# maxwellsh/DIGDriver

Measured on NVIDIA B200. Metric: genome_bases_scanned_per_s, higher is better.
Workload: dtype u8 bases -> int32 counts; f64 p-values

## Files before the change

digdriver_b200/csrc/scan_lb.cu:

```cuda
#include <cuda.h>
#include <string.h>

#include "scan_common.cuh"

using namespace digscan;

namespace {

constexpr int LB_CW = 16;
constexpr int LB_WW = 4;
constexpr int LB_PW = 4;
constexpr int LB_THREADS = (LB_CW + LB_WW + LB_PW) * 32;
constexpr int LB_CONS = LB_CW * 32;
constexpr int LB_SPAN = 128;
constexpr int LB_CHUNK = LB_CW * LB_SPAN;
constexpr uint32_t LB_DSTRIDE = (LB_CHUNK + 64) / 4;
constexpr uint32_t LB_MSTRIDE = (LB_CHUNK + 128) / 8;
constexpr uint32_t LB_DROW = LB_DSTRIDE + 16u;
constexpr uint32_t LB_MROW = LB_MSTRIDE + 16u;
constexpr uint32_t LB_DGROUP = 4u * LB_DROW;
constexpr uint32_t LB_MGROUP = 4u * LB_MROW;
static_assert(LB_DGROUP % 128u == 0u && LB_MGROUP % 128u == 0u, "groups start 128-byte aligned (TMA box destination)");
constexpr uint32_t LB_MBASE = 8u * LB_DGROUP;
constexpr uint32_t LB_STAGE_BYTES = 8u * (LB_DGROUP + LB_MGROUP);
// ... 13 lines not shown
constexpr int LB_NOUT = LB_WW;
constexpr uint32_t OFF_TRI = OFF_OUT + LB_NOUT * OUT_BYTES;
constexpr uint32_t TRI_BYTES = 64u * 33u * 4u;
constexpr uint32_t OFF_EXC = OFF_TRI + TRI_BYTES;
constexpr uint32_t EXC_BYTES = 2048u;
constexpr uint32_t OFF_CNT = OFF_EXC + 2u * EXC_BYTES;
constexpr uint32_t OFF_CHK = OFF_CNT + 256u;
constexpr uint32_t OFF_FLG = OFF_CHK + 128u;
constexpr uint32_t OFF_BAR = OFF_FLG + 16u;
constexpr uint32_t LB_SMEM = OFF_BAR + 256u;
static_assert(OFF_BAR % 16u == 0u, "barrier block alignment");
static_assert(LB_SMEM <= 232448u, "shared memory budget");

constexpr uint32_t LB_BSTAGE = 8u * LB_DGROUP;
constexpr uint32_t OFF_SUM = OFF_STG + 3u * LB_BSTAGE;
static_assert(OFF_SUM + 4u * 128u <= OFF_OUT && LB_BSTAGE <= LB_NOUT * OUT_BYTES, "bases-only ring layout");

enum { BAR_FULL = 0, BAR_EMPTY = 2, BAR_OUTFULL = 4, BAR_OUTEMPTY = 8, BAR_DONE = 12, BAR_CLEAN = 13 };

#ifndef DIG_LB_STAGE3
#define DIG_LB_STAGE3 1
#endif
constexpr bool LB_ST3 = DIG_LB_STAGE3 != 0;
enum { BAR_FULL2 = 14, BAR_EMPTY2 = 15, BAR_OUTFREE = 16, BAR_FULL3 = 17, BAR_EMPTY3 = 18 };
__device__ __forceinline__ uint32_t lb3_full(uint32_t stage)
{
    return stage < 2u ? (uint32_t)BAR_FULL + stage : (stage == 2u ? (uint32_t)BAR_FULL2 : (uint32_t)BAR_FULL3);
}
__device__ __forceinline__ uint32_t lb3_empty(uint32_t stage)
{
    return stage < 2u ? (uint32_t)BAR_EMPTY + stage : (stage == 2u ? (uint32_t)BAR_EMPTY2 : (uint32_t)BAR_EMPTY3);
}
template <bool NS>
struct LbSlots {
    static constexpr uint32_t N = NS ? 4u : 3u;
};
template <bool NS>
__device__ __forceinline__ uint32_t lb_slot(uint32_t stg0, uint32_t stage)
{
    if constexpr (NS) return stage < 3u ? stg0 + stage * LB_BSTAGE : stg0 + (OFF_OUT - OFF_STG);
    else return stg0 + stage * LB_STAGE_BYTES;
}
__device__ __forceinline__ uint32_t lb_slot_sum(uint32_t stg0, uint32_t stage) { return stg0 + (OFF_SUM - OFF_STG) + stage * 128u; }

template <int GM>
struct LbRing {
    static constexpr uint32_t NST = 2u, LOG = 1u, STG0 = OFF_STG, FULL0 = BAR_FULL, EMPTY0 = BAR_EMPTY;
};
constexpr uint32_t TRI_TAB_BYTES = 256u * 128u;
template <>
struct LbRing<2> {
    static constexpr uint32_t NST = 4u, LOG = 2u, STG0 = TRI_TAB_BYTES, FULL0 = 0u, EMPTY0 = 4u;
};
template <>
struct LbRing<3> {
    static constexpr uint32_t NST = 2u, LOG = 1u, STG0 = 0u , FULL0 = 0u, EMPTY0 = 2u;
};
// ... 348 lines not shown

__device__ __forceinline__ int lb_chunk_order(int kq, int nch) { return kq == 0 ? nch - 1 : kq - 1; }

struct LbMaps {
    CUtensorMap d[2], m[2];
};

template <int GM, bool NS>
__device__ __forceinline__ void lb_producer(const LbArgs &A, const LbMaps *maps, const LbTeam T, int pw, int lane)
{
    const uint32_t bar = T.bar;
    const int64_t n_batches = (A.n_reg + 31) >> 5;
    const int m = lane & 3;
    const bool mine = (lane >> T.lane_shift) == pw;
    uint32_t ci = 0u;
    constexpr bool ST3 = LB_ST3 && GM < 2;
    constexpr uint32_t NSL = LbSlots<NS>::N;
    uint32_t uses = 0u, pbi = 0u;
    for (int64_t b = T.b0; b < n_batches; b += T.bstep, ++pbi) {
        const LbGeom g = lb_geom<GM>(b * 32 + lb_win(lane), A.n_reg, A.chrom_off, A.chrom_len, A.reg_chrom, A.reg_start, A.reg_end);
        const int nch = warp_max(g.nch);
        uint32_t st3 = 0u;
        if constexpr (ST3) {
            if (pbi >= 2u) mbar_wait_idle(bar + 8u * BAR_OUTFREE, pbi & 1u);
        }
        const int lead = lane & ~3;
        const uint32_t olo = __shfl_sync(0xffffffffu, (uint32_t)(unsigned long long)g.O, lead);
        const uint32_t ohi = __shfl_sync(0xffffffffu, (uint32_t)((unsigned long long)g.O >> 32), lead);
        const int64_t O0 = (int64_t)(((unsigned long long)ohi << 32) | olo);
        const int n0 = __shfl_sync(0xffffffffu, g.nch, lead);
        const bool fits = A.tile_w > 0 && g.nch > 0 && g.nch == n0 && O0 >= 0 && g.O == O0 + (int64_t)m * 8 * A.tile_w &&
                          g.O + (int64_t)g.nch * LB_CHUNK + 128 <= A.n_bases;
        const uint32_t okm = __ballot_sync(0xffffffffu, fits);
        const bool regular = ((okm >> lead) & 0xFu) == 0xFu;
        const uint32_t ped = (uint32_t)(A.tile_w >> 1), pem = (uint32_t)(A.tile_w >> 2);
        uint32_t xd0 = 0u, yd0 = 0u, xm0 = 0u, ym0 = 0u;
        if (regular && m == 0) {
            const uint32_t ed = (uint32_t)(O0 >> 4), em = (uint32_t)(O0 >> 5);
            yd0 = ed / ped; xd0 = ed - yd0 * ped;
            ym0 = em / pem; xm0 = em - ym0 * pem;
// ... 9 lines not shown
                uses ^= 1u << stage;
                full_i = lb3_full(stage);
                empty_i = lb3_empty(stage);
            } else {
                stage = ci & (R::NST - 1u);
                fpar = (ci >> R::LOG) & 1u;
                full_i = R::FULL0 + stage;
                empty_i = R::EMPTY0 + stage;
            }
            uint32_t sw = 0u;
            if constexpr (NS) {
                if (mine && k < g.nch) sw = lb_span_states(A.nsum, A.n_bases, g.O + (int64_t)k * LB_CHUNK);
            }
            LB_T(t_e0);
            mbar_wait_idle(bar + 8u * empty_i, fpar ^ 1u);
            if constexpr (ST3) {
                if (stage == NSL - 1u && pbi >= 1u) mbar_wait_idle(bar + 8u * BAR_OUTFREE, (pbi - 1u) & 1u);
            }
            LB_T(t_e1);
            const uint32_t full = bar + 8u * full_i;
            const uint32_t stg = ST3 ? lb_slot<NS>(T.stg0, stage) : T.stg0 + stage * LB_STAGE_BYTES;
            if constexpr (NS) {
                if (mine) sts32((ST3 ? lb_slot_sum(T.stg0, stage) : stg + LB_MBASE) + (uint32_t)lb_win(lane) * 4u, sw);
            }
            if (!mine) {
            } else if (regular && k < g.nch) {
                if (m == 0) {
                    uint32_t xd = xd0 + 128u * (uint32_t)k, yd = yd0, xm = xm0 + 64u * (uint32_t)k, ym = ym0;
                    if (xd >= ped) { xd -= ped; ++yd; }
                    if (xm >= pem) { xm -= pem; ++ym; }
                    const int lead = ((lane >> 2) & 1) * 4;
                    int bxd = (int)xd - lead, bxm = (int)xm - lead, sd = 0, sm = 0;
                    if (bxd + (int)(LB_DROW / 4) > (int)ped) { bxd -= (int)A.dshift; sd = 1; }
// ... 33 lines not shown
                    atomicAdd(A.timing + 12, (unsigned long long)(t_i - t_e1));
                }
            }
#endif
        }
    }
}

template <bool TRI, bool NS>
__device__ __forceinline__ void lb_consumer(const LbArgs &A, uint32_t sbase, int warp, int lane)
{
    constexpr uint32_t NSL = LbSlots<NS>::N;
    const uint32_t bar = sbase + OFF_BAR;
    const uint32_t tabl = sbase + OFF_TAB + (uint32_t)lane * 4u;
    const int64_t n_batches = (A.n_reg + 31) >> 5;
    uint32_t cit = 0u, bi = 0u, uses = 0u;
    const uint32_t top_r = A.top | (tabl & A.zero);
    const int grp = warp >> 3, w8 = warp & 7;
#ifdef DIG_LB_TIMING
    unsigned long long tacc[16] = {0, 0, 0, 0, 0, 0, 0, 0, 0, 0, 0, 0, 0, 0, 0, 0};
#endif
    LB_T(t_k0);
    LbGeom gnext = lb_geom<TRI>((int64_t)blockIdx.x * 32 + lb_win(lane), A.n_reg, A.chrom_off, A.chrom_len, A.reg_chrom, A.reg_start, A.reg_end);
    for (int64_t b = blockIdx.x; b < n_batches; b += gridDim.x, ++bi) {
        LB_T(t_g0);
        const LbGeom g = gnext;
        const int nch = warp_max(g.nch);
        LB_T(t_g1);
        LB_ACC(13, t_g0, t_g1);
        const uint32_t par = bi & 1u;
        const uint32_t exc = sbase + OFF_EXC + par * EXC_BYTES;
        uint32_t npairs = 0u;
        bool clean = bi == 0u;
        uint32_t st3 = 0u;
        for (int kq = 0; kq < nch; ++kq, ++cit) {
            const int k = lb_chunk_order(kq, nch);
            uint32_t stage, fpar, full_i, empty_i;
            if constexpr (LB_ST3) {
                stage = st3;
                st3 = st3 == NSL - 1u ? 0u : st3 + 1u;
                fpar = (uses >> stage) & 1u;
                uses ^= 1u << stage;
                full_i = lb3_full(stage);
                empty_i = lb3_empty(stage);
            } else {
                stage = cit & 1u;
                fpar = (cit >> 1) & 1u;
                full_i = BAR_FULL + stage;
                empty_i = BAR_EMPTY + stage;
            }
            LB_T(t_a);
            mbar_wait(bar + 8u * full_i, fpar);
            LB_T(t_b);
            LB_ACC(0, t_a, t_b);
            LB_ACC((kq == 0 ? 8 : (kq == 1 ? 9 : 10)), t_a, t_b);
            const uint32_t stg = LB_ST3 ? lb_slot<NS>(sbase + OFF_STG, stage) : sbase + OFF_STG + stage * LB_STAGE_BYTES;
            {
                const int base0 = k * LB_CHUNK + warp * LB_SPAN;
                const int lo_u = TRI ? min(g.lo5, g.lo3) : g.lo5, hi_u = TRI ? max(g.hi5, g.hi3) : g.hi5;
                if (!__any_sync(0xffffffffu, k < g.nch && lo_u - base0 < 130 && hi_u - base0 > 2)) {
                    if (lane == 0) mbar_arrive(bar + 8u * empty_i);
                    continue;
                }
            }
            const uint32_t dptr = stg + lb_dstrip(lane) + (uint32_t)warp * 32u;
            uint32_t D[9], M[5] = {0u, 0u, 0u, 0u, 0u}, sst = 0u;
            uint32_t dep;
            {
                const uint4 a = lds128(dptr), c = lds128(dptr + 16u);
                D[0] = a.x; D[1] = a.y; D[2] = a.z; D[3] = a.w;
                D[4] = c.x; D[5] = c.y; D[6] = c.z; D[7] = c.w;
                D[8] = lds32(dptr + 32u);
                if constexpr (NS) {
                    const uint32_t sa = LB_ST3 ? lb_slot_sum(sbase + OFF_STG, stage) : stg + LB_MBASE;
                    sst = (lds32(sa + (uint32_t)lb_win(lane) * 4u) >> (2 * warp)) & 3u;
                    dep = (D[0] | D[4]) ^ (D[8] | sst);
                } else {
                    const uint32_t mptr = stg + lb_mstrip(lane) + (uint32_t)warp * 16u;
                    const uint4 m = lds128(mptr);
                    M[0] = m.x; M[1] = m.y; M[2] = m.z; M[3] = m.w;
                    M[4] = lds32(mptr + 16u);
                    dep = (D[0] | D[4]) ^ (D[8] | M[0]) ^ M[4];
                }
            }
            __syncwarp();
            if (lane == 0) mbar_arrive_after_loads(bar + 8u * empty_i, dep, A.zero);
            if (!clean) {
                LB_T(t_c);
                mbar_wait(bar + 8u * BAR_CLEAN, (bi - 1u) & 1u);
                LB_T(t_d);
                LB_ACC(1, t_c, t_d);
                clean = true;
            }
            LB_T(t_p0);
            const int base = k * LB_CHUNK + warp * LB_SPAN;
            const int lo5 = g.lo5 - base, hi5 = g.hi5 - base;
            const uint32_t any_n = NS ? sst : M[0] | M[1] | M[2] | M[3] | (M[4] & 0xF0000000u);
            uint32_t PV[4] = {0u, 0u, 0u, 0u};
#ifdef DIG_LB_UNIFORM_PATH
            if (__all_sync(0xffffffffu, any_n == 0u && lo5 <= 2 && hi5 >= 130)) {
#else
            if (any_n == 0u && lo5 <= 2 && hi5 >= 130) {
#endif
                lb_pairs<false>(D, tabl, A.k32, top_r, PV);
                npairs += 64u;
            } else if (k < g.nch && (!NS || sst != 3u)) {
                if constexpr (NS) {
                    if (sst != 0u) lb_mask_global(A.nmask, A.n_bases, g.O + base, M);
// ... 20 lines not shown
                        if (pos < (uint32_t)LB_EXC_CAP) sts32(exc + 16u + 4u * pos, ((uint32_t)lane << 16) | key);
                    }
                    while (x3) {
                        const int t = __clz(x3);
                        x3 &= ~(0x80000000u >> t);
                        const uint32_t key = lb_bits(D, 32 * j + t + 1, 6);
                        const uint32_t pos = atom_add(exc, 1u);
                        if (pos < (uint32_t)LB_EXC_CAP) sts32(exc + 16u + 4u * pos, ((uint32_t)lane << 16) | 0x8000u | key);
                    }
                }
                if ((PV[0] | PV[1] | PV[2] | PV[3]) != 0u) lb_pairs<true>(D, tabl, A.k32, top_r, PV);
            }
            LB_T(t_p1);
            LB_ACC(2, t_p0, t_p1);
        }
        if (!clean) mbar_wait(bar + 8u * BAR_CLEAN, (bi - 1u) & 1u);
        if (npairs) red_add(sbase + OFF_CNT + par * 128u + (uint32_t)lane * 4u, npairs);
        LB_T(t_s0);
        cons_sync();
        LB_T(t_s1);
        LB_ACC(3, t_s0, t_s1);
        const int64_t rn = (b + gridDim.x) * 32 + lb_win(lane);
        const bool nact = b + gridDim.x < n_batches && rn < A.n_reg;
        int32_t nc = 0;
        int64_t nrs = 0, nre = 0;
        if (nact) {
            nc = __ldg(A.reg_chrom + rn);
            nrs = __ldg(A.reg_start + rn);
            nre = __ldg(A.reg_end + rn);
        }
        mbar_wait(bar + 8u * BAR_DONE, (bi & 1u) ^ 1u);
        LB_T(t_s2);
        LB_ACC(4, t_s1, t_s2);

        uint32_t tri_acc[4] = {0u, 0u, 0u, 0u};
#pragma unroll 1
        for (int i2 = 0; i2 < 4; ++i2) {
          if (i2 == 1) gnext = lb_geom2<TRI>(nact, nc, nrs, nre, A.chrom_off, A.chrom_len);
#pragma unroll
          for (int h = 0; h < 2; ++h) {
            const int i = 2 * i2 + h;
            const int sg = 2 * i + grp;
            const uint32_t buf = (uint32_t)(sg & 3);
            const uint32_t outb = sbase + OFF_OUT + buf * OUT_BYTES + (uint32_t)lb_win(lane) * 256u;
            LB_T(t_w0);
            mbar_wait(bar + 8u * (BAR_OUTEMPTY + buf), (((bi << 2) + (uint32_t)(sg >> 2)) & 1u) ^ 1u);
            LB_T(t_w1);
            LB_ACC(5, t_w0, t_w1);
#pragma unroll
            for (int t = 0; t < 2; ++t) {
                const int jl = (2 * w8 + t + lane) & 15;
                const int j = 16 * sg + jl;
                const uint32_t k0 = lds32(tabl + (uint32_t)(4 * j + 0) * 128u), k1 = lds32(tabl + (uint32_t)(4 * j + 1) * 128u);
                const uint32_t k2 = lds32(tabl + (uint32_t)(4 * j + 2) * 128u), k3 = lds32(tabl + (uint32_t)(4 * j + 3) * 128u);
                const uint32_t w0 = lds32(tabl + (uint32_t)(j)*128u), w1 = lds32(tabl + (uint32_t)(256 + j) * 128u);
                const uint32_t w2 = lds32(tabl + (uint32_t)(512 + j) * 128u), w3 = lds32(tabl + (uint32_t)(768 + j) * 128u);
                const uint32_t a0 = __dp4a(k0, 0x01010101u, 0u), a1 = __dp4a(k1, 0x01010101u, 0u);
                const uint32_t a2 = __dp4a(k2, 0x01010101u, 0u), a3 = __dp4a(k3, 0x01010101u, 0u);
                const uint32_t o0 = __dp4a(w3, 0x01000000u, __dp4a(w2, 0x01000000u, __dp4a(w1, 0x01000000u, __dp4a(w0, 0x01000000u, a0))));
                const uint32_t o2 = __dp4a(w3, 0x00000100u, __dp4a(w2, 0x00000100u, __dp4a(w1, 0x00000100u, __dp4a(w0, 0x00000100u, a2))));
                const uint32_t ev = ((w0 & 0x00FF00FFu) + (w1 & 0x00FF00FFu)) + ((w2 & 0x00FF00FFu) + (w3 & 0x00FF00FFu));
                const uint32_t o1 = a1 + (ev >> 16), o3 = a3 + (ev & 0xFFFFu);
                sts128(outb + (uint32_t)jl * 16u, o0, o1, o2, o3);
                tri_acc[2 * h + t] += (o0 + o1) + (o2 + o3);
            }
            if (i2 == 3) {
                if constexpr (TRI) {
#pragma unroll
                    for (int t = 0; t < 2; ++t) {
                        const uint32_t bin = (uint32_t)(16 * (sg & 3) + ((2 * w8 + t + lane) & 15));
                        red_add(sbase + OFF_TRI + (bin * 33u + (uint32_t)lane) * 4u, tri_acc[2 * h + t]);
                    }
                }
                if (h == 1) red_add(sbase + OFF_CHK + (uint32_t)lane * 4u, (tri_acc[0] + tri_acc[1]) + (tri_acc[2] + tri_acc[3]));
            }
            fence_async();
            __syncwarp();
            if (lane == 0) mbar_arrive(bar + 8u * (BAR_OUTFULL + buf));
            LB_T(t_w2);
            LB_ACC(6, t_w1, t_w2);
          }
        }
    }
#ifdef DIG_LB_TIMING
    LB_T(t_k1);
    LB_ACC(14, t_k0, t_k1);
    if (A.timing != nullptr && lane == 0) {
#pragma unroll
        for (int q = 0; q < 15; ++q)
            if (q != 7 && q != 11 && q != 12) atomicAdd(A.timing + q, tacc[q]);
    }
#endif
}

template <bool TRI, bool TOT>
__device__ __forceinline__ void lb_writer(const LbArgs &A, const CUtensorMap *tmap, uint32_t sbase, int q, int lane)
{
    const uint32_t bar = sbase + OFF_BAR;
    const int64_t n_batches = (A.n_reg + 31) >> 5;
    uint32_t use = 0u, bi = 0u;
    unsigned int tot5[TOT ? 8 : 1], tot3[2] = {0u, 0u};
#pragma unroll
    for (int i = 0; i < (TOT ? 8 : 1); ++i) tot5[i] = 0u;
    unsigned int acc_kb = 0u;
    const uint32_t out = sbase + OFF_OUT + (uint32_t)q * OUT_BYTES;

    auto flush_totals = [&]() {
        if constexpr (TOT) {
#pragma unroll
            for (int i = 0; i < 8; ++i) {
                if (tot5[i]) atomicAdd(A.totals5 + 64 * (4 * (i >> 1) + q) + 2 * lane + (i & 1), (unsigned long long)tot5[i]);
                tot5[i] = 0u;
            }
            if constexpr (TRI) {
                if (tot3[0]) atomicAdd(A.totals3 + lane, (unsigned long long)tot3[0]);
                if (tot3[1]) atomicAdd(A.totals3 + 32 + lane, (unsigned long long)tot3[1]);
                tot3[0] = tot3[1] = 0u;
            }
        }
    };

    for (int64_t b = blockIdx.x; b < n_batches; b += gridDim.x, ++bi) {
        const LbGeom g = lb_geom<TRI>(b * 32 + lb_win(lane), A.n_reg, A.chrom_off, A.chrom_len, A.reg_chrom, A.reg_start, A.reg_end);
        const uint32_t par = bi & 1u;
        const uint32_t exc = sbase + OFF_EXC + par * EXC_BYTES;
        const int64_t r = b * 32 + lb_win(lane);
        unsigned int tmp5[TOT ? 8 : 1], tmp3[2] = {0u, 0u};
#pragma unroll
        for (int i = 0; i < (TOT ? 8 : 1); ++i) tmp5[i] = 0u;
        uint32_t n_exc_raw = 0u;
#pragma unroll
        for (int s4 = 0; s4 < 4; ++s4, ++use) {
            const int sg = 4 * s4 + q;
            mbar_wait_idle(bar + 8u * (BAR_OUTFULL + q), use & 1u);
            if (s4 == 0) n_exc_raw = lds32(exc);
            const uint32_t n_exc = n_exc_raw < (uint32_t)LB_EXC_CAP ? n_exc_raw : (uint32_t)LB_EXC_CAP;
            for (uint32_t e = lane; e < n_exc; e += 32u) {
                const uint32_t ent = lds32(exc + 16u + 4u * e);
                if (!(ent & 0x8000u) && ((ent & 1023u) >> 6) == (uint32_t)sg)
                    red_add(out + (uint32_t)lb_win((int)(ent >> 16)) * 256u + (ent & 63u) * 4u, 1u);
            }
            fence_async();
            __syncwarp();
            if (lane == 0) {
                tensor_s2g(tmap, out, 64 * sg, (int)(b * 32));
                bulk_commit();
            }
            if constexpr (TOT) {
#pragma unroll 8
                for (int l2 = 0; l2 < 32; ++l2) {
                    const uint2 v = lds64(out + (uint32_t)l2 * 256u + (uint32_t)lane * 8u);
                    tmp5[2 * s4] += v.x;
                    tmp5[2 * s4 + 1] += v.y;
                }
            }
            uint32_t dep = 0u;
            if constexpr (TOT) dep = tmp5[2 * s4] | tmp5[2 * s4 + 1];
            __syncwarp();
            if (lane == 0) {
                bulk_wait_read<0>();
                mbar_arrive_after_loads(bar + 8u * (BAR_OUTEMPTY + q), dep, A.zero);
                if constexpr (LB_ST3) {
                    if (s4 == 3) mbar_arrive_after_loads(bar + 8u * BAR_OUTFREE, dep, A.zero);
                }
            }
            __syncwarp();
        }
        writer_sync();
#pragma unroll 8
        for (int i = 0; i < 64; ++i)
            sts128(sbase + OFF_TAB + (uint32_t)q * 32768u + (uint32_t)(lane + 32 * i) * 16u, 0u, 0u, 0u, 0u);
        __threadfence_block();
        __syncwarp();
        if (lane == 0) mbar_arrive(bar + 8u * BAR_CLEAN);
        if (q == 0) {
            const uint32_t n_exc = n_exc_raw < (uint32_t)LB_EXC_CAP ? n_exc_raw : (uint32_t)LB_EXC_CAP;
            if constexpr (TRI) {
                const uint32_t tri = sbase + OFF_TRI;
                for (uint32_t e = lane; e < n_exc; e += 32u) {
                    const uint32_t ent = lds32(exc + 16u + 4u * e);
                    const uint32_t bin = (ent & 0x8000u) ? (ent & 63u) : ((ent >> 2) & 63u);
                    red_add(tri + (bin * 33u + (ent >> 16)) * 4u, 1u);
                }
                __syncwarp();
#pragma unroll 4
                for (int l2 = 0; l2 < 32; ++l2) {
                    const int64_t r2 = b * 32 + lb_win(l2);
                    const uint32_t v0 = lds32(tri + ((uint32_t)lane * 33u + (uint32_t)l2) * 4u);
                    const uint32_t v1 = lds32(tri + ((uint32_t)(lane + 32) * 33u + (uint32_t)l2) * 4u);
                    if (r2 < A.n_reg) {
                        lb_store_tri(A, r2 * 64 + lane, (int)v0);
                        lb_store_tri(A, r2 * 64 + 32 + lane, (int)v1);
                    }
                    tmp3[0] += v0;
                    tmp3[1] += v1;
                }
                __syncwarp();
#pragma unroll 6
                for (int i = 0; i < 66; ++i) sts32(tri + (uint32_t)(lane + 32 * i) * 4u, 0u);
            }
            const uint32_t cnt_a = sbase + OFF_CNT + par * 128u + (uint32_t)lane * 4u, chk_a = sbase + OFF_CHK + (uint32_t)lane * 4u;
            const bool bad = 2u * lds32(cnt_a) != lds32(chk_a);
            const bool fail = __any_sync(0xffffffffu, bad) || n_exc_raw > (uint32_t)LB_EXC_CAP;
            sts32(cnt_a, 0u);
            sts32(chk_a, 0u);
            if (lane == 0) {
                sts32(exc, 0u);
                sts32(sbase + OFF_FLG, fail ? 1u : 0u);
            }
            if (g.too_long || (fail && g.active)) {
                const int pos = atomicAdd(A.fb_count, 1);
                A.fb_list[pos] = (int32_t)r;
            }
        }
        writer_sync();
        const bool fail = lds32(sbase + OFF_FLG) != 0u;
        if constexpr (TOT) {
            if (!fail) {
                unsigned int kb = g.nch > 0 ? (unsigned int)(g.nch * (LB_CHUNK >> 10)) : 0u;
#pragma unroll
                for (int o = 16; o > 0; o >>= 1) kb += __shfl_xor_sync(0xffffffffu, kb, o);
                if (acc_kb + kb > A.tot_limit_kb || acc_kb + kb < acc_kb) {
                    flush_totals();
                    acc_kb = 0u;
                }
                acc_kb += kb;
#pragma unroll
                for (int i = 0; i < 8; ++i) tot5[i] += tmp5[i];
                tot3[0] += tmp3[0];
                tot3[1] += tmp3[1];
            }
        }
        writer_sync();
        if (q == 0 && lane == 0) mbar_arrive(bar + 8u * BAR_DONE);
    }
    flush_totals();
    bulk_wait_all();
}

template <bool PRED>
__device__ __forceinline__ void lb_pairs4(const uint32_t (&D)[9], uint32_t tabl, uint32_t k128, const uint32_t (&PV)[4])
{
#pragma unroll
    for (int i = 0; i < 64; ++i) {
        const int q = i >> 3, off = 4 * (i & 7);
        uint32_t r;
        if (off <= 20) r = D[q] >> (22 - off);
        else r = __funnelshift_r(D[q + 1], D[q], 54 - off);
        uint32_t addr;
        asm("mad.lo.u32 %0, %1, %2, %3;" : "=r"(addr) : "r"(r & 0xFFu), "r"(k128), "r"(tabl));
        if constexpr (!PRED) {
            red_add(addr, 1u);
// ... 275 lines not shown
        const int ww = warp - LB_CW;
        lb_writer_tri<TOT, TEAMS>(A, sbase, ww / L::WW, ww % L::WW, lane);
    } else {
        lb_consumer_tri<TEAMS, NS>(A, sbase, warp / L::CW, warp % L::CW, lane);
    }
}

template <bool TRI, bool TOT, bool NS>
__global__ void __launch_bounds__(LB_THREADS, 1) scan_lb_kernel(const LbArgs A, const __grid_constant__ CUtensorMap tmap,
                                                                const __grid_constant__ LbMaps imaps)
{
    extern __shared__ __align__(1024) unsigned char smem_raw[];
    const uint32_t sbase = (uint32_t)__cvta_generic_to_shared(smem_raw);
    const int lane = threadIdx.x & 31;
    const int warp = __shfl_sync(0xffffffffu, threadIdx.x >> 5, 0);
    if ((sbase & 127u) != 0u) __trap();

    for (uint32_t i = threadIdx.x; i < OFF_BAR / 16u; i += LB_THREADS) sts128(sbase + i * 16u, 0u, 0u, 0u, 0u);
    if (threadIdx.x == 0) {
        const uint32_t bar = sbase + OFF_BAR;
        mbar_init(bar + 8u * (BAR_FULL + 0), 32u);
        mbar_init(bar + 8u * (BAR_FULL + 1), 32u);
        mbar_init(bar + 8u * (BAR_EMPTY + 0), LB_CW);
        mbar_init(bar + 8u * (BAR_EMPTY + 1), LB_CW);
        mbar_init(bar + 8u * BAR_FULL2, 32u);
        mbar_init(bar + 8u * BAR_EMPTY2, LB_CW);
        mbar_init(bar + 8u * BAR_FULL3, 32u);
        mbar_init(bar + 8u * BAR_EMPTY3, LB_CW);
        mbar_init(bar + 8u * BAR_OUTFREE, LB_WW);
#pragma unroll
        for (int i = 0; i < LB_NOUT; ++i) {
            mbar_init(bar + 8u * (BAR_OUTFULL + i), LB_CW / 2);
            mbar_init(bar + 8u * (BAR_OUTEMPTY + i), 1u);
        }
        mbar_init(bar + 8u * BAR_DONE, 1u);
        mbar_init(bar + 8u * BAR_CLEAN, LB_WW);
        asm volatile("fence.mbarrier_init.release.cluster;" ::: "memory");
        fence_async();
    }
    __syncthreads();
    if (warp >= LB_CW + LB_WW)
        lb_producer<TRI, NS>(A, &imaps, LbTeam{(int64_t)blockIdx.x, (int64_t)gridDim.x, sbase + OFF_BAR, sbase + LbRing<TRI>::STG0, 3},
                         warp - LB_CW - LB_WW, lane);
    else if (warp >= LB_CW) lb_writer<TRI, TOT>(A, &tmap, sbase, warp - LB_CW, lane);
    else lb_consumer<TRI, NS>(A, sbase, warp, lane);
}

typedef CUresult (*LbEncodeFn)(CUtensorMap *, CUtensorMapDataType, cuuint32_t, void *, const cuuint64_t *, const cuuint64_t *,
                               const cuuint32_t *, const cuuint32_t *, CUtensorMapInterleave, CUtensorMapSwizzle,
                               CUtensorMapL2promotion, CUtensorMapFloatOOBfill);

int lb_encode(CUtensorMap *tmap, CUtensorMapDataType dtype, const void *base, uint64_t dim0, uint64_t dim1, uint64_t pitch,
              uint32_t box0, uint32_t box1)
{
    static LbEncodeFn encode = nullptr;
    if (encode == nullptr) {
        void *fn = nullptr;
        cudaDriverEntryPointQueryResult q;
        DIG_CUDA(cudaGetDriverEntryPoint("cuTensorMapEncodeTiled", &fn, cudaEnableDefault, &q));
        if (fn == nullptr || q != cudaDriverEntryPointSuccess) {
            dig::set_error("%s: cuTensorMapEncodeTiled is not available", __func__);
            return DIG_ERR_CUDA;
        }
        encode = reinterpret_cast<LbEncodeFn>(fn);
    }
    const cuuint64_t gdim[2] = {dim0, dim1};
    const cuuint64_t gstride[1] = {pitch};
    const cuuint32_t box[2] = {box0, box1};
    const cuuint32_t estride[2] = {1u, 1u};
    const CUresult rc = encode(tmap, dtype, 2u, const_cast<void *>(base), gdim, gstride, box, estride, CU_TENSOR_MAP_INTERLEAVE_NONE,
                               CU_TENSOR_MAP_SWIZZLE_NONE, CU_TENSOR_MAP_L2_PROMOTION_NONE, CU_TENSOR_MAP_FLOAT_OOB_FILL_NONE);
    if (rc != CUDA_SUCCESS) {
        dig::set_error("%s: cuTensorMapEncodeTiled failed (%d)", __func__, (int)rc);
        return DIG_ERR_CUDA;
    }
    return DIG_OK;
}

int lb_tensor_map(CUtensorMap *tmap, int32_t *counts5, int64_t n_reg)
{
    return lb_encode(tmap, CU_TENSOR_MAP_DATA_TYPE_INT32, counts5, 1024u, (uint64_t)n_reg, 4096u, 64u, 32u);
}

int lb_input_maps(LbMaps *maps, LbArgs &A, int64_t tile_w)
{
    A.tile_w = 0;
    A.dshift = A.mshift = 0;
    memset(maps, 0, sizeof(*maps));
    if (tile_w < 4096 || (tile_w & 15) != 0 || tile_w > (int64_t)LB_MAX_CHUNKS * LB_CHUNK || A.n_bases >= ((int64_t)1 << 35))
        return DIG_OK;
    const uint64_t dbytes = (uint64_t)A.n_bases >> 2, mbytes = (uint64_t)A.n_bases >> 3;
    const uint64_t dpitch = 2u * (uint64_t)tile_w, mpitch = (uint64_t)tile_w;
    const uint64_t dsh = (dpitch / 2) & ~(uint64_t)15, msh = (mpitch / 2) & ~(uint64_t)15;
    if (dbytes <= dsh + dpitch || mbytes <= msh + mpitch) return DIG_OK;
    const unsigned char *p2b = reinterpret_cast<const unsigned char *>(A.p2);
    const unsigned char *nmb = reinterpret_cast<const unsigned char *>(A.nmask);
// ... 145 lines not shown
```

Measured before the change: 2828 billion.

## Snapshot count table into tensor memory and let writers reduce from TMEM

Consumers no longer reduce the shared count table into output tiles themselves. After each batch one thread snapshots the table into Blackwell tensor memory with tcgen05.cp, the consumers zero the table, and the writer warps read the counts from TMEM, reduce them and store them through 64B-swizzled TMA tiles. This takes the reduction off the consumer critical path and drops the OUTFULL/OUTEMPTY/CLEAN/OUTFREE handshakes, freeing one ring stage. It also rebalances registers with setmaxnreg and reorganises the exception and totals handling. It relies on one CTA per SM, a 512-column TMEM allocation and new descriptor layouts, and an error there would go unnoticed until the outputs are checked.

Result: slower. 2765 billion (median of 6 runs) (-2.2%).

```diff
diff --git a/digdriver_b200/csrc/lb_tmem.cuh b/digdriver_b200/csrc/lb_tmem.cuh
--- /dev/null
+++ b/digdriver_b200/csrc/lb_tmem.cuh
@@ -0,0 +1,62 @@
+#pragma once
+#include <stdint.h>
+
+namespace lbtmem {
+
+constexpr uint32_t COLS = 512;
+constexpr uint32_t START_COL = 256;
+
+__device__ __forceinline__ void alloc(uint32_t dst_smem)
+{
+    asm volatile("tcgen05.alloc.cta_group::1.sync.aligned.shared::cta.b32 [%0], %1;" ::"r"(dst_smem), "n"(COLS) : "memory");
+    asm volatile("tcgen05.relinquish_alloc_permit.cta_group::1.sync.aligned;" ::: "memory");
+}
+__device__ __forceinline__ void dealloc(uint32_t taddr)
+{
+    asm volatile("tcgen05.dealloc.cta_group::1.sync.aligned.b32 %0, %1;" ::"r"(taddr), "n"(COLS) : "memory");
+}
+__device__ __forceinline__ void fence_before() { asm volatile("tcgen05.fence::before_thread_sync;" ::: "memory"); }
+__device__ __forceinline__ void fence_after() { asm volatile("tcgen05.fence::after_thread_sync;" ::: "memory"); }
+__device__ __forceinline__ void wait_ld() { asm volatile("tcgen05.wait::ld.sync.aligned;" ::: "memory"); }
+
+__device__ __forceinline__ uint64_t desc(uint32_t start, uint32_t lbo, uint32_t sbo)
+{
+    const uint32_t lo = ((start >> 4) & 0x3FFFu) | (((lbo >> 4) & 0x3FFFu) << 16);
+    const uint32_t hi = ((sbo >> 4) & 0x3FFFu) | (1u << 14);
+    return ((uint64_t)hi << 32) | lo;
+}
+__device__ __forceinline__ void cp_128x256b(uint32_t taddr, uint64_t d)
+{
+    asm volatile("tcgen05.cp.cta_group::1.128x256b [%0], %1;" ::"r"(taddr), "l"(d) : "memory");
+}
+
+__device__ __forceinline__ void snapshot(uint32_t tbase, uint32_t tab, uint32_t mbar)
+{
+#pragma unroll 4
+    for (uint32_t c = 0; c < 32u; ++c) {
+        cp_128x256b(tbase + START_COL + 8u * c, desc(tab + 256u * c, 128u, 64u * 128u));
+        cp_128x256b(tbase + 8u * c, desc(tab + 128u * (512u * (c & 1u) + (c >> 1)), 256u * 128u, 16u * 128u));
+    }
+    asm volatile("tcgen05.commit.cta_group::1.mbarrier::arrive::one.shared::cluster.b64 [%0];" ::"r"(mbar) : "memory");
+}
+
+__device__ __forceinline__ void ld16(uint32_t taddr, uint32_t (&v)[16])
+{
+    asm volatile("tcgen05.ld.sync.aligned.32x32b.x16.b32 {%0,%1,%2,%3,%4,%5,%6,%7,%8,%9,%10,%11,%12,%13,%14,%15}, [%16];"
+                 : "=r"(v[0]), "=r"(v[1]), "=r"(v[2]), "=r"(v[3]), "=r"(v[4]), "=r"(v[5]), "=r"(v[6]), "=r"(v[7]), "=r"(v[8]),
+                   "=r"(v[9]), "=r"(v[10]), "=r"(v[11]), "=r"(v[12]), "=r"(v[13]), "=r"(v[14]), "=r"(v[15])
+                 : "r"(taddr)
+                 : "memory");
+}
+
+__device__ __forceinline__ void ld8(uint32_t taddr, uint32_t (&v)[8])
+{
+    asm volatile("tcgen05.ld.sync.aligned.32x32b.x8.b32 {%0,%1,%2,%3,%4,%5,%6,%7}, [%8];"
+                 : "=r"(v[0]), "=r"(v[1]), "=r"(v[2]), "=r"(v[3]), "=r"(v[4]), "=r"(v[5]), "=r"(v[6]), "=r"(v[7])
+                 : "r"(taddr)
+                 : "memory");
+}
+
+__device__ __forceinline__ uint32_t quarter(uint32_t tbase, int q) { return tbase + ((uint32_t)(32 * q) << 16); }
+
+}
diff --git a/digdriver_b200/csrc/scan_lb.cu b/digdriver_b200/csrc/scan_lb.cu
--- a/digdriver_b200/csrc/scan_lb.cu
+++ b/digdriver_b200/csrc/scan_lb.cu
@@ -1,6 +1,7 @@
 #include <cuda.h>
 #include <string.h>
 
+#include "lb_tmem.cuh"
 #include "scan_common.cuh"
 
 using namespace digscan;
@@ -51,33 +52,21 @@
 
 constexpr uint32_t LB_BSTAGE = 8u * LB_DGROUP;
 constexpr uint32_t OFF_SUM = OFF_STG + 3u * LB_BSTAGE;
-static_assert(OFF_SUM + 4u * 128u <= OFF_OUT && LB_BSTAGE <= LB_NOUT * OUT_BYTES, "bases-only ring layout");
-
-enum { BAR_FULL = 0, BAR_EMPTY = 2, BAR_OUTFULL = 4, BAR_OUTEMPTY = 8, BAR_DONE = 12, BAR_CLEAN = 13 };
-
-#ifndef DIG_LB_STAGE3
-#define DIG_LB_STAGE3 1
-#endif
-constexpr bool LB_ST3 = DIG_LB_STAGE3 != 0;
-enum { BAR_FULL2 = 14, BAR_EMPTY2 = 15, BAR_OUTFREE = 16, BAR_FULL3 = 17, BAR_EMPTY3 = 18 };
-__device__ __forceinline__ uint32_t lb3_full(uint32_t stage)
-{
-    return stage < 2u ? (uint32_t)BAR_FULL + stage : (stage == 2u ? (uint32_t)BAR_FULL2 : (uint32_t)BAR_FULL3);
-}
-__device__ __forceinline__ uint32_t lb3_empty(uint32_t stage)
-{
-    return stage < 2u ? (uint32_t)BAR_EMPTY + stage : (stage == 2u ? (uint32_t)BAR_EMPTY2 : (uint32_t)BAR_EMPTY3);
-}
+static_assert(OFF_SUM + 3u * 128u <= OFF_OUT, "bases-only ring layout");
+
+enum { BAR_FULL = 0, BAR_EMPTY = 2, BAR_SNAP = 4, BAR_DONE = 12, BAR_FULL2 = 14, BAR_EMPTY2 = 15 };
+constexpr uint32_t OFF_TADDR = OFF_BAR + 8u * 20u;
+static_assert(OFF_TADDR + 4u <= LB_SMEM, "barrier block");
+static_assert(2u * LB_SMEM > 232448u, "one CTA per SM");
+
+__device__ __forceinline__ uint32_t lb3_full(uint32_t stage) { return stage < 2u ? (uint32_t)BAR_FULL + stage : (uint32_t)BAR_FULL2; }
+__device__ __forceinline__ uint32_t lb3_empty(uint32_t stage) { return stage < 2u ? (uint32_t)BAR_EMPTY + stage : (uint32_t)BAR_EMPTY2; }
 template <bool NS>
 struct LbSlots {
-    static constexpr uint32_t N = NS ? 4u : 3u;
+    static constexpr uint32_t N = NS ? 3u : 2u;
 };
 template <bool NS>
-__device__ __forceinline__ uint32_t lb_slot(uint32_t stg0, uint32_t stage)
-{
-    if constexpr (NS) return stage < 3u ? stg0 + stage * LB_BSTAGE : stg0 + (OFF_OUT - OFF_STG);
-    else return stg0 + stage * LB_STAGE_BYTES;
-}
+__device__ __forceinline__ uint32_t lb_slot(uint32_t stg0, uint32_t stage) { return stg0 + stage * (NS ? LB_BSTAGE : LB_STAGE_BYTES); }
 __device__ __forceinline__ uint32_t lb_slot_sum(uint32_t stg0, uint32_t stage) { return stg0 + (OFF_SUM - OFF_STG) + stage * 128u; }
 
 template <int GM>
@@ -456,16 +445,13 @@
     const int m = lane & 3;
     const bool mine = (lane >> T.lane_shift) == pw;
     uint32_t ci = 0u;
-    constexpr bool ST3 = LB_ST3 && GM < 2;
+    constexpr bool ST3 = GM < 2;
     constexpr uint32_t NSL = LbSlots<NS>::N;
-    uint32_t uses = 0u, pbi = 0u;
-    for (int64_t b = T.b0; b < n_batches; b += T.bstep, ++pbi) {
+    uint32_t uses = 0u;
+    for (int64_t b = T.b0; b < n_batches; b += T.bstep) {
         const LbGeom g = lb_geom<GM>(b * 32 + lb_win(lane), A.n_reg, A.chrom_off, A.chrom_len, A.reg_chrom, A.reg_start, A.reg_end);
         const int nch = warp_max(g.nch);
         uint32_t st3 = 0u;
-        if constexpr (ST3) {
-            if (pbi >= 2u) mbar_wait_idle(bar + 8u * BAR_OUTFREE, pbi & 1u);
-        }
         const int lead = lane & ~3;
         const uint32_t olo = __shfl_sync(0xffffffffu, (uint32_t)(unsigned long long)g.O, lead);
         const uint32_t ohi = __shfl_sync(0xffffffffu, (uint32_t)((unsigned long long)g.O >> 32), lead);
@@ -505,9 +491,6 @@
             }
             LB_T(t_e0);
             mbar_wait_idle(bar + 8u * empty_i, fpar ^ 1u);
-            if constexpr (ST3) {
-                if (stage == NSL - 1u && pbi >= 1u) mbar_wait_idle(bar + 8u * BAR_OUTFREE, (pbi - 1u) & 1u);
-            }
             LB_T(t_e1);
             const uint32_t full = bar + 8u * full_i;
             const uint32_t stg = ST3 ? lb_slot<NS>(T.stg0, stage) : T.stg0 + stage * LB_STAGE_BYTES;
@@ -571,9 +554,8 @@
     const uint32_t bar = sbase + OFF_BAR;
     const uint32_t tabl = sbase + OFF_TAB + (uint32_t)lane * 4u;
     const int64_t n_batches = (A.n_reg + 31) >> 5;
-    uint32_t cit = 0u, bi = 0u, uses = 0u;
+    uint32_t bi = 0u, uses = 0u;
     const uint32_t top_r = A.top | (tabl & A.zero);
-    const int grp = warp >> 3, w8 = warp & 7;
 #ifdef DIG_LB_TIMING
     unsigned long long tacc[16] = {0, 0, 0, 0, 0, 0, 0, 0, 0, 0, 0, 0, 0, 0, 0, 0};
 #endif
@@ -588,30 +570,20 @@
         const uint32_t par = bi & 1u;
         const uint32_t exc = sbase + OFF_EXC + par * EXC_BYTES;
         uint32_t npairs = 0u;
-        bool clean = bi == 0u;
         uint32_t st3 = 0u;
-        for (int kq = 0; kq < nch; ++kq, ++cit) {
+        for (int kq = 0; kq < nch; ++kq) {
             const int k = lb_chunk_order(kq, nch);
-            uint32_t stage, fpar, full_i, empty_i;
-            if constexpr (LB_ST3) {
-                stage = st3;
-                st3 = st3 == NSL - 1u ? 0u : st3 + 1u;
-                fpar = (uses >> stage) & 1u;
-                uses ^= 1u << stage;
-                full_i = lb3_full(stage);
-                empty_i = lb3_empty(stage);
-            } else {
-                stage = cit & 1u;
-                fpar = (cit >> 1) & 1u;
-                full_i = BAR_FULL + stage;
-                empty_i = BAR_EMPTY + stage;
-            }
+            const uint32_t stage = st3;
+            st3 = st3 == NSL - 1u ? 0u : st3 + 1u;
+            const uint32_t fpar = (uses >> stage) & 1u;
+            uses ^= 1u << stage;
+            const uint32_t full_i = lb3_full(stage), empty_i = lb3_empty(stage);
             LB_T(t_a);
             mbar_wait(bar + 8u * full_i, fpar);
             LB_T(t_b);
             LB_ACC(0, t_a, t_b);
             LB_ACC((kq == 0 ? 8 : (kq == 1 ? 9 : 10)), t_a, t_b);
-            const uint32_t stg = LB_ST3 ? lb_slot<NS>(sbase + OFF_STG, stage) : sbase + OFF_STG + stage * LB_STAGE_BYTES;
+            const uint32_t stg = lb_slot<NS>(sbase + OFF_STG, stage);
             {
                 const int base0 = k * LB_CHUNK + warp * LB_SPAN;
                 const int lo_u = TRI ? min(g.lo5, g.lo3) : g.lo5, hi_u = TRI ? max(g.hi5, g.hi3) : g.hi5;
@@ -629,8 +601,7 @@
                 D[4] = c.x; D[5] = c.y; D[6] = c.z; D[7] = c.w;
                 D[8] = lds32(dptr + 32u);
                 if constexpr (NS) {
-                    const uint32_t sa = LB_ST3 ? lb_slot_sum(sbase + OFF_STG, stage) : stg + LB_MBASE;
-                    sst = (lds32(sa + (uint32_t)lb_win(lane) * 4u) >> (2 * warp)) & 3u;
+                    sst = (lds32(lb_slot_sum(sbase + OFF_STG, stage) + (uint32_t)lb_win(lane) * 4u) >> (2 * warp)) & 3u;
                     dep = (D[0] | D[4]) ^ (D[8] | sst);
                 } else {
                     const uint32_t mptr = stg + lb_mstrip(lane) + (uint32_t)warp * 16u;
@@ -642,13 +613,6 @@
             }
             __syncwarp();
             if (lane == 0) mbar_arrive_after_loads(bar + 8u * empty_i, dep, A.zero);
-            if (!clean) {
-                LB_T(t_c);
-                mbar_wait(bar + 8u * BAR_CLEAN, (bi - 1u) & 1u);
-                LB_T(t_d);
-                LB_ACC(1, t_c, t_d);
-                clean = true;
-            }
             LB_T(t_p0);
             const int base = k * LB_CHUNK + warp * LB_SPAN;
             const int lo5 = g.lo5 - base, hi5 = g.hi5 - base;
@@ -699,12 +663,18 @@
             LB_T(t_p1);
             LB_ACC(2, t_p0, t_p1);
         }
-        if (!clean) mbar_wait(bar + 8u * BAR_CLEAN, (bi - 1u) & 1u);
         if (npairs) red_add(sbase + OFF_CNT + par * 128u + (uint32_t)lane * 4u, npairs);
+        fence_async();
         LB_T(t_s0);
         cons_sync();
         LB_T(t_s1);
         LB_ACC(3, t_s0, t_s1);
+        if (warp == 0 && lane == 0) {
+            if (bi > 0u) mbar_wait(bar + 8u * BAR_DONE, (bi - 1u) & 1u);
+            lbtmem::fence_after();
+            lbtmem::snapshot(lds32(sbase + OFF_TADDR), sbase + OFF_TAB, bar + 8u * BAR_SNAP);
+            mbar_arrive(bar + 8u * BAR_SNAP);
+        }
         const int64_t rn = (b + gridDim.x) * 32 + lb_win(lane);
         const bool nact = b + gridDim.x < n_batches && rn < A.n_reg;
         int32_t nc = 0;
@@ -714,58 +684,16 @@
             nrs = __ldg(A.reg_start + rn);
             nre = __ldg(A.reg_end + rn);
         }
-        mbar_wait(bar + 8u * BAR_DONE, (bi & 1u) ^ 1u);
+        gnext = lb_geom2<TRI>(nact, nc, nrs, nre, A.chrom_off, A.chrom_len);
+        mbar_wait(bar + 8u * BAR_SNAP, bi & 1u);
         LB_T(t_s2);
-        LB_ACC(4, t_s1, t_s2);
-
-        uint32_t tri_acc[4] = {0u, 0u, 0u, 0u};
-#pragma unroll 1
-        for (int i2 = 0; i2 < 4; ++i2) {
-          if (i2 == 1) gnext = lb_geom2<TRI>(nact, nc, nrs, nre, A.chrom_off, A.chrom_len);
-#pragma unroll
-          for (int h = 0; h < 2; ++h) {
-            const int i = 2 * i2 + h;
-            const int sg = 2 * i + grp;
-            const uint32_t buf = (uint32_t)(sg & 3);
-            const uint32_t outb = sbase + OFF_OUT + buf * OUT_BYTES + (uint32_t)lb_win(lane) * 256u;
-            LB_T(t_w0);
-            mbar_wait(bar + 8u * (BAR_OUTEMPTY + buf), (((bi << 2) + (uint32_t)(sg >> 2)) & 1u) ^ 1u);
-            LB_T(t_w1);
-            LB_ACC(5, t_w0, t_w1);
-#pragma unroll
-            for (int t = 0; t < 2; ++t) {
-                const int jl = (2 * w8 + t + lane) & 15;
-                const int j = 16 * sg + jl;
-                const uint32_t k0 = lds32(tabl + (uint32_t)(4 * j + 0) * 128u), k1 = lds32(tabl + (uint32_t)(4 * j + 1) * 128u);
-                const uint32_t k2 = lds32(tabl + (uint32_t)(4 * j + 2) * 128u), k3 = lds32(tabl + (uint32_t)(4 * j + 3) * 128u);
-                const uint32_t w0 = lds32(tabl + (uint32_t)(j)*128u), w1 = lds32(tabl + (uint32_t)(256 + j) * 128u);
-                const uint32_t w2 = lds32(tabl + (uint32_t)(512 + j) * 128u), w3 = lds32(tabl + (uint32_t)(768 + j) * 128u);
-                const uint32_t a0 = __dp4a(k0, 0x01010101u, 0u), a1 = __dp4a(k1, 0x01010101u, 0u);
-                const uint32_t a2 = __dp4a(k2, 0x01010101u, 0u), a3 = __dp4a(k3, 0x01010101u, 0u);
-                const uint32_t o0 = __dp4a(w3, 0x01000000u, __dp4a(w2, 0x01000000u, __dp4a(w1, 0x01000000u, __dp4a(w0, 0x01000000u, a0))));
-                const uint32_t o2 = __dp4a(w3, 0x00000100u, __dp4a(w2, 0x00000100u, __dp4a(w1, 0x00000100u, __dp4a(w0, 0x00000100u, a2))));
-                const uint32_t ev = ((w0 & 0x00FF00FFu) + (w1 & 0x00FF00FFu)) + ((w2 & 0x00FF00FFu) + (w3 & 0x00FF00FFu));
-                const uint32_t o1 = a1 + (ev >> 16), o3 = a3 + (ev & 0xFFFFu);
-                sts128(outb + (uint32_t)jl * 16u, o0, o1, o2, o3);
-                tri_acc[2 * h + t] += (o0 + o1) + (o2 + o3);
-            }
-            if (i2 == 3) {
-                if constexpr (TRI) {
-#pragma unroll
-                    for (int t = 0; t < 2; ++t) {
-                        const uint32_t bin = (uint32_t)(16 * (sg & 3) + ((2 * w8 + t + lane) & 15));
-                        red_add(sbase + OFF_TRI + (bin * 33u + (uint32_t)lane) * 4u, tri_acc[2 * h + t]);
-                    }
-                }
-                if (h == 1) red_add(sbase + OFF_CHK + (uint32_t)lane * 4u, (tri_acc[0] + tri_acc[1]) + (tri_acc[2] + tri_acc[3]));
-            }
-            fence_async();
-            __syncwarp();
-            if (lane == 0) mbar_arrive(bar + 8u * (BAR_OUTFULL + buf));
-            LB_T(t_w2);
-            LB_ACC(6, t_w1, t_w2);
-          }
-        }
+        LB_ACC(1, t_s1, t_s2);
+#pragma unroll 4
+        for (int i = 0; i < 16; ++i)
+            sts128(sbase + OFF_TAB + (uint32_t)warp * 8192u + (uint32_t)(lane + 32 * i) * 16u, 0u, 0u, 0u, 0u);
+        cons_sync();
+        LB_T(t_s3);
+        LB_ACC(4, t_s2, t_s3);
     }
 #ifdef DIG_LB_TIMING
     LB_T(t_k1);
@@ -778,88 +706,139 @@
 #endif
 }
 
+__device__ __forceinline__ uint32_t lb_swz64(uint32_t a) { return a ^ (((a >> 7) & 3u) << 4); }
+__device__ __forceinline__ uint32_t lb_reduce4(const uint32_t (&cs)[4], int lane)
+{
+    const bool b2 = lane & 4, b1 = lane & 2;
+    uint32_t u[2];
+#pragma unroll
+    for (int k = 0; k < 2; ++k) u[k] = (b2 ? cs[k + 2] : cs[k]) + __shfl_xor_sync(0xffffffffu, b2 ? cs[k] : cs[k + 2], 4);
+    const uint32_t w = (b1 ? u[1] : u[0]) + __shfl_xor_sync(0xffffffffu, b1 ? u[0] : u[1], 2);
+    return w + __shfl_xor_sync(0xffffffffu, w, 1);
+}
+
 template <bool TRI, bool TOT>
-__device__ __forceinline__ void lb_writer(const LbArgs &A, const CUtensorMap *tmap, uint32_t sbase, int q, int lane)
+__device__ __forceinline__ void lb_writer(const LbArgs &A, const CUtensorMap *tmap, uint32_t sbase, uint32_t tbase, int q, int lane)
 {
     const uint32_t bar = sbase + OFF_BAR;
     const int64_t n_batches = (A.n_reg + 31) >> 5;
-    uint32_t use = 0u, bi = 0u;
+    uint32_t bi = 0u;
     unsigned int tot5[TOT ? 8 : 1], tot3[2] = {0u, 0u};
 #pragma unroll
     for (int i = 0; i < (TOT ? 8 : 1); ++i) tot5[i] = 0u;
     unsigned int acc_kb = 0u;
+    const int gg = lane >> 3, li = lane & 7, g = 4 * q + gg;
+    const int lbin = 4 * (lane & 1) + 2 * ((lane >> 2) & 1) + ((lane >> 1) & 1);
+    const uint32_t tq = lbtmem::quarter(tbase, q);
     const uint32_t out = sbase + OFF_OUT + (uint32_t)q * OUT_BYTES;
+    const uint32_t tile = out + (uint32_t)gg * (OUT_BYTES / 4u);
+#ifdef DIG_LB_TIMING
+    unsigned long long t_idle = 0ull, t_busy = 0ull;
+#endif
 
     auto flush_totals = [&]() {
         if constexpr (TOT) {
 #pragma unroll
-            for (int i = 0; i < 8; ++i) {
-                if (tot5[i]) atomicAdd(A.totals5 + 64 * (4 * (i >> 1) + q) + 2 * lane + (i & 1), (unsigned long long)tot5[i]);
-                tot5[i] = 0u;
+            for (int p = 0; p < 8; ++p) {
+                if (tot5[p]) atomicAdd(A.totals5 + 64 * g + 8 * p + lbin, (unsigned long long)tot5[p]);
+                tot5[p] = 0u;
             }
             if constexpr (TRI) {
-                if (tot3[0]) atomicAdd(A.totals3 + lane, (unsigned long long)tot3[0]);
-                if (tot3[1]) atomicAdd(A.totals3 + 32 + lane, (unsigned long long)tot3[1]);
+                if (q == 0) {
+                    if (tot3[0]) atomicAdd(A.totals3 + lane, (unsigned long long)tot3[0]);
+                    if (tot3[1]) atomicAdd(A.totals3 + 32 + lane, (unsigned long long)tot3[1]);
+                }
                 tot3[0] = tot3[1] = 0u;
             }
         }
     };
 
     for (int64_t b = blockIdx.x; b < n_batches; b += gridDim.x, ++bi) {
-        const LbGeom g = lb_geom<TRI>(b * 32 + lb_win(lane), A.n_reg, A.chrom_off, A.chrom_len, A.reg_chrom, A.reg_start, A.reg_end);
         const uint32_t par = bi & 1u;
         const uint32_t exc = sbase + OFF_EXC + par * EXC_BYTES;
-        const int64_t r = b * 32 + lb_win(lane);
+        LB_T(t_w0);
+        mbar_wait_idle(bar + 8u * BAR_SNAP, par);
+        LB_T(t_w1);
+        lbtmem::fence_after();
+        const uint32_t n_exc_raw = lds32(exc);
+        const uint32_t n_exc = n_exc_raw < (uint32_t)LB_EXC_CAP ? n_exc_raw : (uint32_t)LB_EXC_CAP;
         unsigned int tmp5[TOT ? 8 : 1], tmp3[2] = {0u, 0u};
 #pragma unroll
         for (int i = 0; i < (TOT ? 8 : 1); ++i) tmp5[i] = 0u;
-        uint32_t n_exc_raw = 0u;
-#pragma unroll
-        for (int s4 = 0; s4 < 4; ++s4, ++use) {
-            const int sg = 4 * s4 + q;
-            mbar_wait_idle(bar + 8u * (BAR_OUTFULL + q), use & 1u);
-            if (s4 == 0) n_exc_raw = lds32(exc);
-            const uint32_t n_exc = n_exc_raw < (uint32_t)LB_EXC_CAP ? n_exc_raw : (uint32_t)LB_EXC_CAP;
+#pragma unroll 1
+        for (int k = 0; k < 4; ++k) {
+            uint32_t chk[4] = {0u, 0u, 0u, 0u};
+            uint32_t rt[2] = {0u, 0u};
+#pragma unroll
+            for (int yl = 0; yl < 4; ++yl) {
+                const int y = 4 * k + yl;
+                uint32_t V[16];
+                lbtmem::ld16(tq + lbtmem::START_COL + 16u * (uint32_t)y, V);
+                lbtmem::wait_ld();
+#pragma unroll
+                for (int j = 0; j < 16; ++j) V[j] = __dp4a(V[j], 0x01010101u, 0u);
+#pragma unroll
+                for (int h = 0; h < 2; ++h) {
+                    uint32_t E[8];
+                    lbtmem::ld8(tq + 16u * (uint32_t)y + 8u * (uint32_t)h, E);
+                    lbtmem::wait_ld();
+#pragma unroll
+                    for (int f = 0; f < 4; ++f)
+#pragma unroll
+                        for (int e = 0; e < 4; ++e)
+                            V[4 * f + e] = __dp4a(E[e], 1u << (8 * (3 - f)), __dp4a(E[4 + e], 1u << (8 * (3 - f)), V[4 * f + e]));
+                }
+                if (yl == 0) {
+                    if (lane == 0) bulk_wait_read<0>();
+                    __syncwarp();
+                }
+                uint32_t cs[4] = {0u, 0u, 0u, 0u};
+#pragma unroll
+                for (int e = 0; e < 4; ++e) {
+                    const uint32_t o[4] = {V[e], V[4 + e], V[8 + e], V[12 + e]};
+                    sts128(lb_swz64(tile + (uint32_t)(li + 8 * e) * 64u + (uint32_t)yl * 16u), o[0], o[1], o[2], o[3]);
+                    const uint32_t t = (o[0] + o[1]) + (o[2] + o[3]);
+                    chk[e] += t;
+                    if constexpr (TRI) red_add(sbase + OFF_TRI + ((uint32_t)(16 * gg + y) * 33u + (uint32_t)(4 * li + e)) * 4u, t);
+                    if constexpr (TOT) {
+#pragma unroll
+                        for (int f = 0; f < 4; ++f) cs[f] += o[f];
+                    }
+                }
+                if constexpr (TOT) {
+                    const uint32_t v = lb_reduce4(cs, lane);
+                    rt[yl >> 1] += (lane & 1) == (yl & 1) ? v : 0u;
+                }
+            }
+            __syncwarp();
             for (uint32_t e = lane; e < n_exc; e += 32u) {
-                const uint32_t ent = lds32(exc + 16u + 4u * e);
-                if (!(ent & 0x8000u) && ((ent & 1023u) >> 6) == (uint32_t)sg)
-                    red_add(out + (uint32_t)lb_win((int)(ent >> 16)) * 256u + (ent & 63u) * 4u, 1u);
+                const uint32_t ent = lds32(exc + 16u + 4u * e), m = ent & 1023u;
+                if (!(ent & 0x8000u) && (m >> 8) == (uint32_t)q && ((m >> 4) & 3u) == (uint32_t)k)
+                    red_add(lb_swz64(out + ((m >> 6) & 3u) * (OUT_BYTES / 4u) + (uint32_t)lb_win((int)(ent >> 16)) * 64u + ((m >> 2) & 3u) * 16u) +
+                                (m & 3u) * 4u,
+                            1u);
             }
             fence_async();
             __syncwarp();
             if (lane == 0) {
-                tensor_s2g(tmap, out, 64 * sg, (int)(b * 32));
+#pragma unroll
+                for (int t = 0; t < 4; ++t) tensor_s2g(tmap, out + (uint32_t)t * (OUT_BYTES / 4u), 64 * (4 * q + t) + 16 * k, (int)(b * 32));
                 bulk_commit();
             }
+#pragma unroll
+            for (int e = 0; e < 4; ++e) red_add(sbase + OFF_CHK + (uint32_t)(4 * li + e) * 4u, chk[e]);
             if constexpr (TOT) {
-#pragma unroll 8
-                for (int l2 = 0; l2 < 32; ++l2) {
-                    const uint2 v = lds64(out + (uint32_t)l2 * 256u + (uint32_t)lane * 8u);
-                    tmp5[2 * s4] += v.x;
-                    tmp5[2 * s4 + 1] += v.y;
-                }
-            }
-            uint32_t dep = 0u;
-            if constexpr (TOT) dep = tmp5[2 * s4] | tmp5[2 * s4 + 1];
-            __syncwarp();
-            if (lane == 0) {
-                bulk_wait_read<0>();
-                mbar_arrive_after_loads(bar + 8u * (BAR_OUTEMPTY + q), dep, A.zero);
-                if constexpr (LB_ST3) {
-                    if (s4 == 3) mbar_arrive_after_loads(bar + 8u * BAR_OUTFREE, dep, A.zero);
-                }
-            }
-            __syncwarp();
-        }
+#pragma unroll
+                for (int p = 0; p < 6; ++p) tmp5[p] = tmp5[p + 2];
+                tmp5[6] = rt[0];
+                tmp5[7] = rt[1];
+            }
+        }
+        lbtmem::fence_before();
         writer_sync();
-#pragma unroll 8
-        for (int i = 0; i < 64; ++i)
-            sts128(sbase + OFF_TAB + (uint32_t)q * 32768u + (uint32_t)(lane + 32 * i) * 16u, 0u, 0u, 0u, 0u);
-        __threadfence_block();
-        __syncwarp();
-        if (lane == 0) mbar_arrive(bar + 8u * BAR_CLEAN);
+        const int64_t r = b * 32 + lb_win(lane);
+        const LbGeom geo = lb_geom<TRI>(r, A.n_reg, A.chrom_off, A.chrom_len, A.reg_chrom, A.reg_start, A.reg_end);
         if (q == 0) {
-            const uint32_t n_exc = n_exc_raw < (uint32_t)LB_EXC_CAP ? n_exc_raw : (uint32_t)LB_EXC_CAP;
             if constexpr (TRI) {
                 const uint32_t tri = sbase + OFF_TRI;
                 for (uint32_t e = lane; e < n_exc; e += 32u) {
@@ -889,20 +868,30 @@
             const bool fail = __any_sync(0xffffffffu, bad) || n_exc_raw > (uint32_t)LB_EXC_CAP;
             sts32(cnt_a, 0u);
             sts32(chk_a, 0u);
+            if constexpr (TOT) {
+                if (!fail) {
+                    for (uint32_t e = lane; e < n_exc; e += 32u) {
+                        const uint32_t ent = lds32(exc + 16u + 4u * e);
+                        if (!(ent & 0x8000u)) atomicAdd(A.totals5 + (ent & 1023u), 1ull);
+                    }
+                }
+            }
             if (lane == 0) {
                 sts32(exc, 0u);
                 sts32(sbase + OFF_FLG, fail ? 1u : 0u);
             }
-            if (g.too_long || (fail && g.active)) {
+            if (geo.too_long || (fail && geo.active)) {
                 const int pos = atomicAdd(A.fb_count, 1);
                 A.fb_list[pos] = (int32_t)r;
             }
+            __syncwarp();
+            if (lane == 0) mbar_arrive(bar + 8u * BAR_DONE);
         }
         writer_sync();
         const bool fail = lds32(sbase + OFF_FLG) != 0u;
         if constexpr (TOT) {
             if (!fail) {
-                unsigned int kb = g.nch > 0 ? (unsigned int)(g.nch * (LB_CHUNK >> 10)) : 0u;
+                unsigned int kb = geo.nch > 0 ? (unsigned int)(geo.nch * (LB_CHUNK >> 10)) : 0u;
 #pragma unroll
                 for (int o = 16; o > 0; o >>= 1) kb += __shfl_xor_sync(0xffffffffu, kb, o);
                 if (acc_kb + kb > A.tot_limit_kb || acc_kb + kb < acc_kb) {
@@ -916,11 +905,26 @@
                 tot3[1] += tmp3[1];
             }
         }
-        writer_sync();
-        if (q == 0 && lane == 0) mbar_arrive(bar + 8u * BAR_DONE);
+#ifdef DIG_LB_TIMING
+        LB_T(t_w2);
+        t_idle += (unsigned long long)(t_w1 - t_w0);
+        t_busy += (unsigned long long)(t_w2 - t_w1);
+#endif
     }
     flush_totals();
-    bulk_wait_all();
+    if (lane == 0) bulk_wait_all();
+#ifdef DIG_LB_TIMING
+    if (A.timing != nullptr && lane == 0) {
+        atomicAdd(A.timing + 5, t_idle);
+        atomicAdd(A.timing + 6, t_busy);
+    }
+#endif
+    lbtmem::fence_before();
+    writer_sync();
+    if (q == 0) {
+        lbtmem::fence_after();
+        lbtmem::dealloc(tbase);
+    }
 }
 
 template <bool PRED>
@@ -1226,7 +1230,7 @@
     const uint32_t sbase = (uint32_t)__cvta_generic_to_shared(smem_raw);
     const int lane = threadIdx.x & 31;
     const int warp = __shfl_sync(0xffffffffu, threadIdx.x >> 5, 0);
-    if ((sbase & 127u) != 0u) __trap();
+    if ((sbase & 511u) != 0u) __trap();
 
     for (uint32_t i = threadIdx.x; i < OFF_BAR / 16u; i += LB_THREADS) sts128(sbase + i * 16u, 0u, 0u, 0u, 0u);
     if (threadIdx.x == 0) {
@@ -1237,25 +1241,25 @@
         mbar_init(bar + 8u * (BAR_EMPTY + 1), LB_CW);
         mbar_init(bar + 8u * BAR_FULL2, 32u);
         mbar_init(bar + 8u * BAR_EMPTY2, LB_CW);
-        mbar_init(bar + 8u * BAR_FULL3, 32u);
-        mbar_init(bar + 8u * BAR_EMPTY3, LB_CW);
-        mbar_init(bar + 8u * BAR_OUTFREE, LB_WW);
-#pragma unroll
-        for (int i = 0; i < LB_NOUT; ++i) {
-            mbar_init(bar + 8u * (BAR_OUTFULL + i), LB_CW / 2);
-            mbar_init(bar + 8u * (BAR_OUTEMPTY + i), 1u);
-        }
+        mbar_init(bar + 8u * BAR_SNAP, 2u);
         mbar_init(bar + 8u * BAR_DONE, 1u);
-        mbar_init(bar + 8u * BAR_CLEAN, LB_WW);
         asm volatile("fence.mbarrier_init.release.cluster;" ::: "memory");
         fence_async();
     }
+    if (warp == LB_CW) lbtmem::alloc(sbase + OFF_TADDR);
+    lbtmem::fence_before();
     __syncthreads();
-    if (warp >= LB_CW + LB_WW)
+    lbtmem::fence_after();
+    if (warp >= LB_CW + LB_WW) {
+        asm volatile("setmaxnreg.dec.sync.aligned.u32 48;" ::: "memory");
         lb_producer<TRI, NS>(A, &imaps, LbTeam{(int64_t)blockIdx.x, (int64_t)gridDim.x, sbase + OFF_BAR, sbase + LbRing<TRI>::STG0, 3},
-                         warp - LB_CW - LB_WW, lane);
-    else if (warp >= LB_CW) lb_writer<TRI, TOT>(A, &tmap, sbase, warp - LB_CW, lane);
-    else lb_consumer<TRI, NS>(A, sbase, warp, lane);
+                             warp - LB_CW - LB_WW, lane);
+    } else if (warp >= LB_CW) {
+        asm volatile("setmaxnreg.inc.sync.aligned.u32 112;" ::: "memory");
+        lb_writer<TRI, TOT>(A, &tmap, sbase, lds32(sbase + OFF_TADDR), warp - LB_CW, lane);
+    } else {
+        lb_consumer<TRI, NS>(A, sbase, warp, lane);
+    }
 }
 
 typedef CUresult (*LbEncodeFn)(CUtensorMap *, CUtensorMapDataType, cuuint32_t, void *, const cuuint64_t *, const cuuint64_t *,
@@ -1263,7 +1267,7 @@
                                CUtensorMapL2promotion, CUtensorMapFloatOOBfill);
 
 int lb_encode(CUtensorMap *tmap, CUtensorMapDataType dtype, const void *base, uint64_t dim0, uint64_t dim1, uint64_t pitch,
-              uint32_t box0, uint32_t box1)
+              uint32_t box0, uint32_t box1, CUtensorMapSwizzle swizzle = CU_TENSOR_MAP_SWIZZLE_NONE)
 {
     static LbEncodeFn encode = nullptr;
     if (encode == nullptr) {
@@ -1281,7 +1285,7 @@
     const cuuint32_t box[2] = {box0, box1};
     const cuuint32_t estride[2] = {1u, 1u};
     const CUresult rc = encode(tmap, dtype, 2u, const_cast<void *>(base), gdim, gstride, box, estride, CU_TENSOR_MAP_INTERLEAVE_NONE,
-                               CU_TENSOR_MAP_SWIZZLE_NONE, CU_TENSOR_MAP_L2_PROMOTION_NONE, CU_TENSOR_MAP_FLOAT_OOB_FILL_NONE);
+                               swizzle, CU_TENSOR_MAP_L2_PROMOTION_NONE, CU_TENSOR_MAP_FLOAT_OOB_FILL_NONE);
     if (rc != CUDA_SUCCESS) {
         dig::set_error("%s: cuTensorMapEncodeTiled failed (%d)", __func__, (int)rc);
         return DIG_ERR_CUDA;
@@ -1291,7 +1295,7 @@
 
 int lb_tensor_map(CUtensorMap *tmap, int32_t *counts5, int64_t n_reg)
 {
-    return lb_encode(tmap, CU_TENSOR_MAP_DATA_TYPE_INT32, counts5, 1024u, (uint64_t)n_reg, 4096u, 64u, 32u);
+    return lb_encode(tmap, CU_TENSOR_MAP_DATA_TYPE_INT32, counts5, 1024u, (uint64_t)n_reg, 4096u, 16u, 32u, CU_TENSOR_MAP_SWIZZLE_64B);
 }
 
 int lb_input_maps(LbMaps *maps, LbArgs &A, int64_t tile_w)
```
